# vlad17/runlmc

Measured on AMD Instinct MI355X. Metric: kronecker_toeplitz_mvms_per_sec, higher is better.
Workload: dtype f64

## Files before the change

runlmc_amd/csrc/rl_gridop.hip:

```cpp
#include "rl_host.h"

static thread_local std::string g_err;

int fail(int code, const std::string& msg) {
    g_err = msg;
    return code;
}

extern "C" const char* rl_last_error(void) { return g_err.c_str(); }
extern "C" const char* rl_backend(void) { return RL_BACKEND_NAME; }
extern "C" int rl_abi_version(void) { return RL_ABI_VERSION; }
extern "C" int rl_device_count(int* count) {
    if (!count) return fail(RL_EINVAL, "count is NULL");
    RL_HIP(hipGetDeviceCount(count));
    return RL_OK;
}

void trace_once(const char* what) {
    static const bool on = getenv("RUNLMC_TRACE") != nullptr;
    if (!on) return;
    static std::vector<std::string> seen;
    for (const std::string& s : seen)
        if (s == what) return;
    seen.push_back(what);
// ... 1 lines not shown
}

bool first_on_device(unsigned long long* seen) {
    int dev = 0;
    (void)hipGetDevice(&dev);
    const unsigned long long bit = 1ull << (dev & 63);
    if (*seen & bit) return false;
    *seen |= bit;
    return true;
}

RlKnobs read_knobs() {
    RlKnobs k;
    const char* dbg = getenv("RUNLMC_DEBUG");
    const bool debug = dbg != nullptr && dbg[0] != '\0' && dbg[0] != '0';
    auto ignored = [](const char* n) {
        static std::vector<std::string> told;
        if (std::find(told.begin(), told.end(), std::string(n)) == told.end()) {
            told.push_back(n);
            fprintf(stderr, "runlmc_hip: %s is a debug switch and is ignored without RUNLMC_DEBUG=1\n", n);
        }
    };
    auto user_flag = [](const char* n) { return getenv(n) != nullptr; };
    auto user_num = [](const char* n, long long dflt) {
        const char* e = getenv(n);
        return e ? atoll(e) : dflt;
    };
    auto flag = [&](const char* n) {
        if (getenv(n) == nullptr) return false;
        if (!debug) ignored(n);
        return debug;
    };
    auto num = [&](const char* n, long long dflt) {
        const char* e = getenv(n);
        if (e == nullptr) return dflt;
        if (!debug) ignored(n);
        return debug ? atoll(e) : dflt;
    };
    k.pow2_only = user_flag("RUNLMC_POW2_ONLY");
    k.chunk_mb = (int)num("RUNLMC_CHUNK_MB", 0);
    k.two_streams = (int)num("RUNLMC_TWO_STREAMS", -1);
    k.affine = (int)num("RUNLMC_AFFINE", -1);
    k.affine_kb = (int)num("RUNLMC_AFFINE_KB", 0);
    k.affine_max_kb = (int)num("RUNLMC_AFFINE_MAX_KB", 2048);
    k.no_v1p = flag("RUNLMC_NO_V1P");
    k.v1p_min = (int)num("RUNLMC_V1P_MIN", 0);
    k.no_lowrank = flag("RUNLMC_NO_LOWRANK");
    k.no_filter = flag("RUNLMC_NO_FILTER");
    k.no_lr_bound = flag("RUNLMC_NO_LR_BOUND");
    k.sf_carries1 = flag("RUNLMC_SF_CARRIES1");
    k.sf_scan2 = flag("RUNLMC_SF_SCAN2");
    k.poly_round = flag("RUNLMC_POLY_ROUND");
    k.no_poly_round = flag("RUNLMC_NO_POLY_ROUND");
    k.lr_min = num("RUNLMC_LR_MIN", -1);
    k.staged_wt = flag("RUNLMC_STAGED_WT");
    k.no_staged_wt = flag("RUNLMC_NO_STAGED_WT");
    k.no_w_poly = flag("RUNLMC_NO_W_POLY");
    k.no_rp = flag("RUNLMC_NO_RP");
    k.rp_stagger = (int)num("RUNLMC_RP_STAGGER", 7);
    k.no_lr_small = flag("RUNLMC_NO_LR_SMALL");
    k.no_precond_approx = flag("RUNLMC_NO_PRECOND_APPROX");
    k.no_precond_hi = flag("RUNLMC_NO_PRECOND_HI");
    k.precond_hi_passes = flag("RUNLMC_PRECOND_HI_PASSES");
    k.no_precond_hi_mixed = flag("RUNLMC_NO_PRECOND_HI_MIXED");
    k.precond_hi_min = num("RUNLMC_PRECOND_HI_MIN", 100000);
    k.precond_hi_rank = (int)num("RUNLMC_PRECOND_HI_RANK", 192);
    k.precond_hi_use = (int)num("RUNLMC_PRECOND_HI_USE", 0);
    k.rp_fly = (int)num("RUNLMC_RP_FLY", 1);
    k.no_rp_small = flag("RUNLMC_NO_RP_SMALL");
    k.no_rp_fuse = flag("RUNLMC_NO_RP_FUSE");
    k.rp_pfuse = !flag("RUNLMC_NO_RP_PFUSE");
    k.w_pfuse = !flag("RUNLMC_NO_W_PFUSE");
    k.rp_runlen = (int)num("RUNLMC_RP_RUNLEN", 0);
    k.w_poly_rmax = std::min(36, (int)num("RUNLMC_W_POLY_RMAX", 32));
    k.no_sort = flag("RUNLMC_NO_SORT");
    k.ws_cache_mb = user_num("RUNLMC_WS_CACHE_MB", -1);
    k.solver_maxblk = (int)num("RUNLMC_SOLVER_MAXBLK", 0);
    k.no_fuse_w = flag("RUNLMC_NO_FUSE_W");
    k.no_fuse_wt = flag("RUNLMC_NO_FUSE_WT");
    k.no_graph = flag("RUNLMC_NO_GRAPH");
#if defined(RL_EMU)
    k.minres_v1 = flag("RUNLMC_MINRES_V1");
#endif
    return k;
}

static int ilog2(int x) {
    int l = 0;
    while ((1 << l) < x) ++l;
    return l;
}

static FftPlan make_plan(int n) {
    FftPlan p;
    p.n = n;
    p.npass = 0;
    for (int i = 0; i < RL_MAX_PASSES; ++i) p.radix[i] = 1;
    int rem = n;
    for (int odd : {3, 5})
        while (rem % odd == 0 && p.npass < 2) {
            p.radix[p.npass++] = odd;
            rem /= odd;
        }
    const int fixed[7][4] = {{8, 8, 0, 0},     {16, 16, 0, 0},   {64, 8, 8, 0},
                             {128, 8, 16, 0},  {256, 16, 16, 0}, {512, 8, 8, 8},
                             {1024, 8, 8, 16}};
    for (const auto& f : fixed)
        if (f[0] == rem) {
            for (int i = 1; i < 4 && f[i]; ++i) p.radix[p.npass++] = f[i];
            return p;
        }
    while (rem > 1) {
        int r = 8;
        while (rem % r) r /= 2;
        p.radix[p.npass++] = r;
        rem /= r;
    }
    return p;
}

static bool make_plan_rows3(int n, FftPlan* p) {
    int ra, rb;
    switch (n) {
        case 128: ra = 8; rb = 8; break;
        case 256: ra = 16; rb = 8; break;
        case 512: ra = 16; rb = 16; break;
        default: return false;
    }
    p->n = n;
    p->npass = 3;
    for (int i = 0; i < RL_MAX_PASSES; ++i) p->radix[i] = 1;
    p->radix[0] = ra;
    p->radix[1] = rb;
    p->radix[2] = 2;
    return true;
}

static int fused_code(const FftPlan& p) {
    if (p.npass < 2 || p.npass > 4) return 0;
    const int ra = p.radix[0], rb = p.radix[p.npass - 1];
    const int code = ra * 100 + rb;
    switch (code) {
        case 808: case 816: case 1616: return p.n >= 64 ? code : 0;
        case 308: case 316: case 508: case 516: return code;
        default: return 0;
    }
}

static void choose_length(int m, bool pow2_only, int* L_out, int* N1_out, int* N2_out) {
    long best = 0;
    int best_odd = 1;
    for (int odd : {1, 3, 5, 9, 15, 25}) {
        if (odd != 1 && pow2_only) continue;
        long L = odd;
        while (L < 2L * m || L < 16) L *= 2;
        if (odd != 1 && L / odd < 64 * 8) continue;
        if (best == 0 || L < best) { best = L; best_odd = odd; }
    }
    const int L = (int)best;
    const int P = L / best_odd;
    const int l = ilog2(P);
    int N2 = 1 << ((l + 1) / 2);
    if (best_odd != 1) {
        int bestN2 = 0;
        double bestScore = 1e300;
        for (int n2 = 64; n2 <= 1024 && n2 <= P / 8; n2 *= 2) {
// ... 274 lines not shown
    if (((size_t)g->N1 * C + g->N1) * sizeof(cplx) > kLdsHard)
        return fail(RL_ELIMIT, "rl_gridop_create: grid too long for one LDS column tile");
    g->colsA = C;

    g->plan1 = make_plan(g->N1);
    g->plan2 = make_plan(g->N2);
    g->code1 = fused_code(g->plan1);
    g->code2 = fused_code(g->plan2);
    bool rows_ok = g->code2 == 808 || g->code2 == 816 || g->code2 == 1616;
    if (g->code1 != 0 &&
        (size_t)g->N2 * D * sizeof(cplx) <= kLdsHard && make_plan_rows3(g->N2, &g->plan2)) {
        g->rows3 = true;
        g->code2 = g->plan2.radix[0] * 100 + g->plan2.radix[1];
        rows_ok = true;
    }
    g->v2 = g->code1 != 0 && rows_ok;
    g->lr_try = m1 == 0 && m >= 2 * RL_LR_RMAX && m < (1 << 28) && !g->kn.no_lowrank;
    g->lr_round_try = g->lr_try && (m >= 2048 || g->kn.poly_round);
    g->sf_try = m1 == 0 && m >= 64 && !g->kn.no_filter;
    g->lr_min = lr_min_elements(g);
    g->h_freq1 = position_to_freq(g->plan1);
    g->h_freq2 = position_to_freq(g->plan2);

    int rc;
    if ((rc = upload(&g->tw1, unity_table(g->N1, 1, g->N1))) != RL_OK) return rc;
    if ((rc = upload(&g->tw2, unity_table(g->N2, 1, g->N2))) != RL_OK) return rc;
    const int shift = l / 2;
    if ((rc = upload(&g->twlo, unity_table(1L << shift, 1, L))) != RL_OK) return rc;
    if ((rc = upload(&g->twhi, unity_table(((long)L + (1L << shift) - 1) >> shift, 1L << shift,
                                           L))) != RL_OK) return rc;
    if ((rc = upload(&g->freq1, g->h_freq1)) != RL_OK) return rc;
    g->twl.lo = m1 == 0 ? g->twlo : nullptr;
    g->twl.hi = g->twhi;
    g->twl.shift = shift;
    g->twl.mask = (1 << shift) - 1;

    g->max_fac = max_tops * D;
    RL_HIP(hipMalloc((void**)&g->tops, (size_t)max_tops * m * sizeof(double)));
    RL_HIP(hipMalloc((void**)&g->spec, (size_t)max_tops * L * sizeof(double)));
    RL_HIP(hipMalloc((void**)&g->facA, (size_t)g->max_fac * D * sizeof(double)));
    RL_HIP(hipMalloc((void**)&g->facW, (size_t)g->max_fac * sizeof(double)));
    RL_HIP(hipMalloc((void**)&g->facQ, (size_t)g->max_fac * sizeof(int)));
    RL_HIP(hipMalloc((void**)&g->kappa, (size_t)max_tops * D * sizeof(double)));
    std::vector<double> ones(D, 1.0);
    if ((rc = upload(&g->ones, ones)) != RL_OK) return rc;

    size_t chunk_mb = (size_t)D * L * sizeof(cplx) >= ((size_t)8 << 20) ? 64 : 192;
    if (g->kn.chunk_mb > 0) chunk_mb = (size_t)g->kn.chunk_mb;
    g->chunk_pairs = std::max<size_t>(1, (chunk_mb << 20) / ((size_t)D * L * sizeof(cplx)));
    {
        const size_t pairT = (size_t)D * L * sizeof(cplx);
        const bool can = g->v2 && g->rows3 && m1 == 0;
        g->affine = can && (g->kn.affine >= 0 ? g->kn.affine != 0
                                              : (pairT >= ((size_t)512 << 10) &&
                                                 pairT <= ((size_t)g->kn.affine_max_kb << 10)));
        if (g->affine && g->kn.affine_kb > 0 && g->kn.chunk_mb <= 0)
            g->chunk_pairs = 8 * std::max<size_t>(1, ((size_t)g->kn.affine_kb << 10) / pairT);
    }
    if (m1 == 0 && L <= 2048 && !g->kn.no_v1p) {
        const size_t lds = ((size_t)L * (D | 1) + L) * sizeof(cplx);
        if (lds <= kLdsHard) {
            g->planL = make_plan(L);
            if ((rc = upload(&g->twL, unity_table(L, 1, L))) != RL_OK) return rc;
            RL_HIP(hipMalloc((void**)&g->spec1, (size_t)max_tops * L * sizeof(double)));
            g->lds1 = lds;
            g->thr1 = (size_t)D * L >= 4096 ? 512 : 256;
            g->v1p = true;
            if (g->kn.v1p_min > 0) g->v1p_min = g->kn.v1p_min;
        }
    }
    *out = guard.release();
    return RL_OK;
}

extern "C" int rl_gridop_destroy(rl_gridop* g) {
    if (!g) return RL_OK;
    (void)hipSetDevice(g->device);
    if (g->child) (void)rl_gridop_destroy(g->child);
    if (g->wide_B) (void)hipFree(g->wide_B);
    if (g->wide_Z) (void)hipFree(g->wide_Z);
    void* ptrs[] = {g->tw1, g->tw2, g->twlo, g->twhi, g->freq1, g->tops, g->spec,
                    g->facA, g->facW, g->facQ, g->kappa, g->ones, g->T,
                    g->T2[0], g->T2[1], g->T2[2], g->twL, g->spec1, g->mixtab, g->lr_beta, g->lr_nu, g->lr_phiJ, g->lr_stat, g->lr_M,
                    g->lr_B, g->lr_eye, g->lr_part, g->lr_zhat, g->lr_scr, g->lr_pw, g->lr_sel, g->lr_Cc, g->lr_Bc, g->lr_Mf, g->lr_spart, g->lr_Cx,
                    g->sf_tops, g->sf_blob, g->sf_blob_top, g->sf_pwp, g->sf_pw, g->sf_kappa, g->sf_facA, g->sf_facAW, g->sf_facJ,
                    g->sf_E, g->sf_Cin, g->sf_next};
    for (void* p : ptrs)
        if (p) (void)hipFree(p);
    if (g->ev_fork) (void)hipEventDestroy(g->ev_fork);
    for (int i = 0; i < 3; ++i) {
        if (g->ev_join[i]) (void)hipEventDestroy(g->ev_join[i]);
        if (g->aux[i]) (void)hipStreamDestroy(g->aux[i]);
    }
    delete g;
    return RL_OK;
}

extern "C" int rl_gridop_info(const rl_gridop* g, int* L, int* N1, int* N2, int* colsA,
                              int* rowsB) {
    if (!g) return fail(RL_EINVAL, "gridop is NULL");
    if (L) *L = g->L;
    if (N1) *N1 = g->N1;
    if (N2) *N2 = g->N2;
    if (colsA) *colsA = g->colsA;
    if (rowsB) *rowsB = g->rowsB;
    return RL_OK;
}

extern "C" int rl_gridop_form(const rl_gridop* gc, int* rank, long long* min_elements) {
    if (!gc) return fail(RL_EINVAL, "gridop is NULL");
    if (gc->wide) {
        return rl_gridop_form(gc->child, rank, min_elements);
    }
    rl_gridop* g = const_cast<rl_gridop*>(gc);
    if (g->Q >= 1) RL_TRY(lr_ensure(g));
    if (rank) *rank = g->lr_ok ? g->lr_r : 0;
    if (min_elements) *min_elements = (long long)g->lr_min;
    return RL_OK;
}

extern "C" int rl_gridop_top_forms(const rl_gridop* gc, int* forms, int* structured) {
    if (!gc) return fail(RL_EINVAL, "gridop is NULL");
    if (gc->wide) {
        RL_TRY(rl_gridop_top_forms(gc->child, forms, nullptr));
        if (structured) {
            *structured = 1;
            for (int q = 0; q < gc->child->Q; ++q)
                if (gc->child->top_form[q] == 0) *structured = 0;
        }
        return RL_OK;
    }
    rl_gridop* g = const_cast<rl_gridop*>(gc);
    if (g->Q < 1) return fail(RL_EINVAL, "grid operator has no parameters yet");
    RL_TRY(lr_ensure(g));
    if (forms)
        for (int q = 0; q < g->Q; ++q)
            forms[q] = q < (int)g->top_form.size() ? g->top_form[q] : 0;
    if (structured) *structured = (g->lr_ok || g->st_ok) ? 1 : 0;
    return RL_OK;
}

extern "C" int rl_gridop_form_stats(const rl_gridop* gc, int q, double* out4) {
    if (!gc || !out4) return fail(RL_EINVAL, "rl_gridop_form_stats: NULL argument");
    if (gc->wide) return rl_gridop_form_stats(gc->child, q, out4);
    rl_gridop* g = const_cast<rl_gridop*>(gc);
    if (g->Q < 1) return fail(RL_EINVAL, "grid operator has no parameters yet");
    if (q < 0 || q >= g->Q) return fail(RL_EINVAL, "rl_gridop_form_stats: no such top row");
    RL_TRY(lr_ensure(g));
    for (int k = 0; k < 4; ++k)
        out4[k] = (size_t)(4 * q + k) < g->lr_vstat.size() ? g->lr_vstat[4 * q + k] : 0.0;
    return RL_OK;
}

extern "C" int rl_gridop_set_form_gate(rl_gridop* g, long long min_elements) {
    if (!g) return fail(RL_EINVAL, "gridop is NULL");
    if (g->wide) return rl_gridop_set_form_gate(g->child, min_elements);
    g->lr_min = min_elements < 0 ? lr_min_elements(g) : (size_t)min_elements;
    return RL_OK;
}

static int build_spectra(rl_gridop* g, int ntop, hipStream_t stream) {
    const int npairs = (ntop + 1) / 2;
    const size_t need = ((size_t)npairs + g->D - 1) / g->D;
    RL_TRY(ensure_workspace(g, std::max<size_t>(need, 1)));
    dim3 gridA(g->N2 / g->colsA, 1, npairs);
    Gather no_gather;
    no_gather.indptr = nullptr;
// ... 495 lines not shown
    std::vector<double> phiJ((size_t)(R + 16) * m, 0.0), beta(R), nu(R);
    std::vector<long double> prev(m, 0.0L), cur(m), nxt(m);
    const long double p0 = 1.0L / sqrtl((long double)m);
    for (int n = 0; n < m; ++n) cur[n] = p0;
    long double bj = 0.0L, nuj = p0;
    for (int j = 0; j < R + RL_LR_EXTRA; ++j) {
        for (int n = 0; n < m; ++n) phiJ[(size_t)j * m + n] = (double)cur[n];
        if (j < R) {
            beta[j] = (double)(bj * bj);
            nu[j] = (double)nuj;
        }
        long double nrm = 0.0L;
        for (int n = 0; n < m; ++n) {
            const long double sn = m > 1 ? -1.0L + 2.0L * n / (m - 1) : 0.0L;
            nxt[n] = sn * cur[n] - bj * prev[n];
            nrm += nxt[n] * nxt[n];
        }
        bj = sqrtl(nrm);
        if (!(bj > 0.0L)) return fail(RL_EINVAL, "polynomial basis degenerate");
        nuj /= bj;
        for (int n = 0; n < m; ++n) {
            prev[n] = cur[n];
            cur[n] = nxt[n] / bj;
        }
    }
    RL_TRY(upload(&g->lr_phiJ, phiJ));
    RL_TRY(upload(&g->lr_beta, beta));
    RL_TRY(upload(&g->lr_nu, nu));
    g->lr_hnu = nu;
    return RL_OK;
}

static int lr_steps(const rl_gridop* g, int nrows, int R) {
    const int slots = (g->m + 1) / 2;
    if (slots <= 64 * RL_LR_T) return std::max(4, ((slots + 63) / 64 + 3) / 4 * 4);
    const int rowblocks = (nrows + RL_LR_ROWS(R) - 1) / RL_LR_ROWS(R);
    const double resident = 2.0 * RL_LR_CUS;
    int best = RL_LR_T;
    double best_cost = 1e300;
    for (int steps = RL_LR_T; steps <= 8 * RL_LR_T; steps *= 2) {
        const int chunks = ((g->m + 1) / 2 + 64 * steps - 1) / (64 * steps);
        const double rounds = std::ceil((double)chunks * rowblocks / resident);
        const double cost = rounds * (steps + 8);
        if (cost < best_cost * 0.97) {
            best_cost = cost;
            best = steps;
        }
        if (chunks == 1) break;
    }
    return best;
}
static int lr_nchunks_max(const rl_gridop* g) {
    return ((g->m + 1) / 2 + 64 * RL_LR_T - 1) / (64 * RL_LR_T);
}
static size_t lr_part_need(const rl_gridop* g, int nvec) {
    return (size_t)lr_nchunks_max(g) * nvec * g->D * RL_LR_RMAX;
}
int lr_reserve(rl_gridop* g, int nvec) {
    const size_t rows = (size_t)nvec * g->D;
    const size_t need_part = lr_part_need(g, nvec), need_z = rows * RL_LR_RMAX;
    if (g->lr_part_cap < need_part) {
        if (g->lr_part) RL_HIP(hipFree(g->lr_part));
        g->lr_part = nullptr;
        g->lr_part_cap = 0;
        RL_HIP(hipMalloc((void**)&g->lr_part, need_part * sizeof(double)));
        g->lr_part_cap = need_part;
    }
    if (g->lr_zhat_cap < need_z) {
        if (g->lr_zhat) RL_HIP(hipFree(g->lr_zhat));
        g->lr_zhat = nullptr;
        g->lr_zhat_cap = 0;
        RL_HIP(hipMalloc((void**)&g->lr_zhat, need_z * sizeof(double)));
        g->lr_zhat_cap = need_z;
    }
    return RL_OK;
}

static size_t lr_min_elements(const rl_gridop* g) {
    return g->kn.lr_min >= 0 ? (size_t)g->kn.lr_min : (size_t)1 << 20;
}

template <int R>
static int lr_project(rl_gridop* g, const double* X, int nrows, hipStream_t st,
                      double* part = nullptr) {
    const int steps = lr_steps(g, nrows, R);
    const int chunks = ((g->m + 1) / 2 + 64 * steps - 1) / (64 * steps);
    RL_LAUNCH((k_lr_project<R>), dim3(chunks, (nrows + RL_LR_ROWS(R) - 1) / RL_LR_ROWS(R)),
              dim3(64 * RL_LR_WAVES), (size_t)RL_LR_WAVES * R * 65 * sizeof(double), st, X, nrows,
              g->m, (const double*)g->lr_beta, steps, part != nullptr ? part : g->lr_part);
    return chunks;
}
template <int R>
static void lr_mix(rl_gridop* g, const double* part, int chunks, int nvec, int Q, const double* Cq,
                   const double* Bq, double* zhat, hipStream_t st) {
    int split3 = 0;
    const size_t mix_lds = lr_mix_lds(g->D, R, Q, &split3);
    RL_LAUNCH(k_lr_mix, dim3(nvec), dim3(RL_LR_MIXT), mix_lds, st, part, chunks, nvec, g->D, R, Q,
              Cq, Bq, (const double*)g->lr_nu, zhat, (const int*)nullptr, split3);
}
template <int R>
static void lr_expand(rl_gridop* g, const double* zhat, int nrows, double* Y, int accumulate,
                      hipStream_t st) {
    const int per_cu = 8;
    const int nbx = ((g->m + 1) / 2 + 255) / 256;
    int rpb = 16;
    if ((size_t)nbx * ((nrows + 15) / 16) < (size_t)2 * per_cu * RL_LR_CUS) {
        const int nby = std::max(1, std::min(nrows, per_cu * RL_LR_CUS / nbx));
        rpb = (nrows + nby - 1) / nby;
    }
    if (accumulate)
        RL_LAUNCH((k_lr_expand<R, true>), dim3(nbx, (nrows + rpb - 1) / rpb), dim3(256), 0,
                  st, zhat, nrows, g->m, (const double*)g->lr_beta, rpb, Y);
    else
        RL_LAUNCH((k_lr_expand<R, false>), dim3(nbx, (nrows + rpb - 1) / rpb), dim3(256), 0,
                  st, zhat, nrows, g->m, (const double*)g->lr_beta, rpb, Y);
}
template <int R>
static void lr_launch(rl_gridop* g, const double* X, double* Y, int nvec, int Q, const double* Cq,
                      const double* Bq, hipStream_t st, int accumulate = 0) {
    const int nrows = nvec * g->D;
    const bool deferred = g->defer_expand && !accumulate && R <= g->kn.w_poly_rmax;
    const int chunks = lr_project<R>(g, X, nrows, st);
    lr_mix<R>(g, g->lr_part, chunks, nvec, Q, Cq, Bq, g->lr_zhat, st);
    if (deferred) {
        g->expand_deferred = true;
        return;
    }
    lr_expand<R>(g, g->lr_zhat, nrows, Y, accumulate, st);
}

static int lr_apply(rl_gridop* g, const double* X, double* Y, int nvec, int q0, int Q,
                    const double* Bq, hipStream_t st) {
    const double* Cq = g->lr_C + (size_t)q0 * g->lr_r * g->lr_r;
    switch (g->lr_r) {
        case 24: lr_launch<24>(g, X, Y, nvec, Q, Cq, Bq, st); break;
        case 32: lr_launch<32>(g, X, Y, nvec, Q, Cq, Bq, st); break;
        case 36: lr_launch<36>(g, X, Y, nvec, Q, Cq, Bq, st); break;
        case 40: lr_launch<40>(g, X, Y, nvec, Q, Cq, Bq, st); break;
        case 48: lr_launch<48>(g, X, Y, nvec, Q, Cq, Bq, st); break;
        default: return fail(RL_EINVAL, "low-rank path: bad basis size");
    }
    RL_HIP(hipGetLastError());
    return RL_OK;
}

static int lr_apply_compact(rl_gridop* g, const double* X, double* Y, int nvec, hipStream_t st) {
    switch (g->lr_r) {
        case 24: lr_launch<24>(g, X, Y, nvec, g->lr_np, g->lr_Cc, g->lr_Bc, st, 1); break;
        case 32: lr_launch<32>(g, X, Y, nvec, g->lr_np, g->lr_Cc, g->lr_Bc, st, 1); break;
        case 36: lr_launch<36>(g, X, Y, nvec, g->lr_np, g->lr_Cc, g->lr_Bc, st, 1); break;
        case 40: lr_launch<40>(g, X, Y, nvec, g->lr_np, g->lr_Cc, g->lr_Bc, st, 1); break;
        case 48: lr_launch<48>(g, X, Y, nvec, g->lr_np, g->lr_Cc, g->lr_Bc, st, 1); break;
        default: return fail(RL_EINVAL, "low-rank path: bad basis size");
    }
    RL_HIP(hipGetLastError());
    return RL_OK;
}

static int mvm_with_mix(rl_gridop* g, const MixParams& mp, const double* X, double* Y, int nvec,
                        hipStream_t stream);

struct SfFit {
    int deg = 0;
    long double ah = 0.0L;
    long double c[3] = {0.0L, 0.0L, 0.0L};
};

static bool sf_check(const double* t, int m, const SfFit& f, long double tot) {
// ... 252 lines not shown
            red[512 + tid] += red[512 + tid + s];
        }
        __syncthreads();
    }
    if (tid == 0) {
        out[blockIdx.x * 3 + 0] = red[0];
        out[blockIdx.x * 3 + 1] = red[256];
        out[blockIdx.x * 3 + 2] = red[512];
    }
}
__global__ void __launch_bounds__(256)
k_lr_rowmax(const double* __restrict__ V, int m, double* __restrict__ out) {
    RL_SMEM(smem);
    double* red = reinterpret_cast<double*>(smem);
    const double* v = V + (size_t)blockIdx.x * m;
    double mx = 0.0;
    for (int i = threadIdx.x; i < m; i += 256) {
        const double a = fabs(v[i]);
        mx = (a > mx || !(a <= 1e300)) ? a : mx;
    }
    const int tid = threadIdx.x;
    red[tid] = mx;
    __syncthreads();
    for (int s = 128; s > 0; s >>= 1) {
        if (tid < s) {
            const double o = red[tid + s];
            if (o > red[tid] || !(o <= 1e300)) red[tid] = o;
        }
        __syncthreads();
    }
    if (tid == 0) out[blockIdx.x] = red[0];
}
#define RL_LR_NPOW 8
#define RL_LR_TOL_OP 2e-13
#if defined(RL_EMU)
#define RL_LR_PWB 8
#else
#define RL_LR_PWB 512
#endif
__global__ void __launch_bounds__(256)
k_lr_pw_diff(const double* a, const double* b, int m, double* out, double* __restrict__ part) {
    RL_SMEM(smem);
    double* red = reinterpret_cast<double*>(smem);
    const size_t off = (size_t)blockIdx.y * m;
    double s = 0.0;
    for (int i = blockIdx.x * 256 + threadIdx.x; i < m; i += gridDim.x * 256) {
        const double d = b ? a[off + i] - b[off + i] : a[off + i];
        out[off + i] = d;
        s = fma(d, d, s);
    }
    const int tid = threadIdx.x;
    red[tid] = s;
    __syncthreads();
    for (int w = 128; w > 0; w >>= 1) {
        if (tid < w) red[tid] += red[tid + w];
        __syncthreads();
    }
    if (tid == 0) part[(size_t)blockIdx.y * gridDim.x + blockIdx.x] = red[0];
}
__global__ void __launch_bounds__(256)
k_lr_pw_scale(const double* __restrict__ d, int m, const double* __restrict__ part,
              double* __restrict__ v, double* __restrict__ stat, const int* __restrict__ top_of_row,
              int stride, int off) {
    RL_SMEM(smem);
    double* red = reinterpret_cast<double*>(smem);
    const int row = blockIdx.y, tid = threadIdx.x;
    double sp = 0.0;
    for (int b = tid; b < (int)gridDim.x; b += 256) sp += part[(size_t)row * gridDim.x + b];
    red[tid] = sp;
    __syncthreads();
    for (int w = 128; w > 0; w >>= 1) {
        if (tid < w) red[tid] += red[tid + w];
        __syncthreads();
    }
    const double nrm = sqrt(red[0]);
    const double inv = (nrm > 0.0 && nrm <= 1e300) ? 1.0 / nrm : 1.0;
    const size_t o = (size_t)row * m;
    for (int i = blockIdx.x * 256 + threadIdx.x; i < m; i += gridDim.x * 256) v[o + i] = d[o + i] * inv;
    if (blockIdx.x == 0 && threadIdx.x == 0 && top_of_row[row] >= 0)
        stat[(size_t)top_of_row[row] * stride + off] = nrm;
}
#define RL_LR_STATW (RL_LR_NB * 3 + RL_LR_RMAX + 16 + 2 * RL_LR_NPOW)

static int lr_verify(rl_gridop* g, const std::vector<char>& want, std::vector<char>* pass) {
    const int D = g->D, m = g->m, Q = g->Q;
    const size_t vec = (size_t)D * m;
    pass->assign(Q, 0);
    if (!g->lr_phiJ) {
        RL_TRY(lr_make_basis(g));
        double* cs = nullptr;
        RL_HIP(hipMalloc((void**)&cs, (size_t)g->max_tops * (RL_LR_STATW + RL_LR_RMAX * RL_LR_RMAX) * sizeof(double)));
        RL_HIP(hipMemset(cs, 0, (size_t)g->max_tops * (RL_LR_STATW + RL_LR_RMAX * RL_LR_RMAX) * sizeof(double)));
        g->lr_stat = cs;
        g->lr_C = cs + (size_t)g->max_tops * RL_LR_STATW;
        RL_HIP(hipMalloc((void**)&g->lr_Cc, (size_t)g->max_tops * RL_LR_RMAX * RL_LR_RMAX * sizeof(double)));
        RL_HIP(hipMalloc((void**)&g->lr_B, (size_t)g->max_tops * D * D * sizeof(double)));
        RL_HIP(hipMalloc((void**)&g->lr_Bc, (size_t)g->max_tops * D * D * sizeof(double)));
        std::vector<double> eye((size_t)D * D, 0.0);
        for (int a = 0; a < D; ++a) eye[(size_t)a * D + a] = 1.0;
        RL_TRY(upload(&g->lr_eye, eye));
        const size_t nvr = (RL_LR_RMAX + RL_LR_EXTRA + D - 1) / D;
        RL_HIP(hipMalloc((void**)&g->lr_scr, (3 + nvr) * vec * sizeof(double)));
        RL_HIP(hipMalloc((void**)&g->lr_pw, (4 * vec + 2 * (size_t)RL_LR_PWB * D) * sizeof(double)));
        RL_HIP(hipMalloc((void**)&g->lr_sel, (size_t)g->max_tops *
                         ((size_t)g->max_tops * D + (size_t)g->max_tops * D * D + D) * sizeof(double)));
        std::vector<double> xr(vec);
        unsigned long long st = 0x9E3779B97F4A7C15ull;
        for (size_t i = 0; i < vec; ++i) {
            st = st * 6364136223846793005ull + 1442695040888963407ull;
            xr[i] = ((double)(st >> 11) / 9007199254740992.0) * 2.0 - 1.0;
        }
        for (int a = 0; a < D; ++a) {
            long double ss = 0.0L;
            for (int i = 0; i < m; ++i) ss += (long double)xr[(size_t)a * m + i] * xr[(size_t)a * m + i];
            const double inv = ss > 0.0L ? (double)(1.0L / sqrtl(ss)) : 1.0;
            for (int i = 0; i < m; ++i) xr[(size_t)a * m + i] *= inv;
        }
        RL_HIP(hipMemcpy(g->lr_scr, xr.data(), vec * sizeof(double), hipMemcpyHostToDevice));
    }
    double* xr = g->lr_scr;
    double* y1 = xr + vec;
    double* y2 = y1 + vec;
    double* tphi = y2 + vec;
    hipStream_t st = nullptr;
    std::vector<double> back;
    std::vector<char> best;
    std::vector<int> cand;
    for (int q = 0; q < Q; ++q)
        if (want[q]) cand.push_back(q);
    const size_t sel_stride = (size_t)Q * D + (size_t)Q * D * D + D;
    {
        const size_t ngroups = (cand.size() + D - 1) / D;
        std::vector<double> sel(std::max<size_t>(1, ngroups) * sel_stride, 0.0);
        for (size_t grp = 0; grp < ngroups; ++grp) {
            double* ks = sel.data() + grp * sel_stride;
            double* bs = ks + (size_t)Q * D;
            int* rows = reinterpret_cast<int*>(bs + (size_t)Q * D * D);
            for (int a = 0; a < D; ++a) rows[a] = -1;
            for (int a = 0; a < D && grp * D + a < cand.size(); ++a) {
                const int q = cand[grp * D + a];
                ks[(size_t)q * D + a] = 1.0;
                bs[((size_t)q * D + a) * D + a] = 1.0;
                rows[a] = q;
            }
        }
        RL_HIP(hipMemcpy(g->lr_sel, sel.data(), sel.size() * sizeof(double), hipMemcpyHostToDevice));
    }
    for (int r : {24, 32, 36, 40, 48}) {
        if (r < g->lr_rank_hint && r < 48) continue;
        g->lr_r = r;
        const int nvr = (r + RL_LR_EXTRA + D - 1) / D, nrows = nvr * D;
        RL_TRY(lr_reserve(g, std::max(nvr, 1)));
        RL_HIP(hipMemsetAsync(g->lr_C, 0, (size_t)g->max_tops * RL_LR_RMAX * RL_LR_RMAX * sizeof(double), st));
        for (int q = 0; q < Q; ++q) {
            if (!want[q]) continue;
            MixParams mp{1, 0, g->spec + (size_t)q * g->L, nullptr, nullptr, nullptr, g->ones,
                         nullptr, nullptr};
            double* stat = g->lr_stat + (size_t)q * RL_LR_STATW;
            g->lr_bypass = true;
            int rc = mvm_with_mix(g, mp, g->lr_phiJ, tphi, nvr, st);
            g->lr_bypass = false;
            if (rc != RL_OK) return rc;
            RL_LAUNCH(k_lr_rowmax, dim3(nrows), dim3(256), 256 * sizeof(double), st,
                      (const double*)tphi, m, stat + RL_LR_NB * 3);
            int nparts = 0;
            switch (r) {
                case 24: nparts = lr_project<24>(g, tphi, nrows, st); break;
                case 32: nparts = lr_project<32>(g, tphi, nrows, st); break;
                case 36: nparts = lr_project<36>(g, tphi, nrows, st); break;
                case 40: nparts = lr_project<40>(g, tphi, nrows, st); break;
                default: nparts = lr_project<48>(g, tphi, nrows, st); break;
            }
            RL_LAUNCH(k_lr_finish_C, dim3(r), dim3(256), 512 * sizeof(double), st,
                      (const double*)g->lr_part, nparts, nrows, r, (const double*)g->lr_nu,
                      g->lr_C + (size_t)q * r * r);
            g->lr_bypass = true;
            rc = mvm_with_mix(g, mp, xr, y1, 1, st);
            g->lr_bypass = false;
            if (rc != RL_OK) return rc;
            RL_TRY(lr_apply(g, xr, y2, 1, q, 1, g->lr_eye, st));
            RL_LAUNCH(k_lr_compare, dim3(RL_LR_NB), dim3(256), 3 * 256 * sizeof(double), st,
                      (const double*)y1, (const double*)y2, vec, stat);
        }
        for (size_t grp = 0; grp * D < cand.size(); ++grp) {
            double* vw = g->lr_pw;
            double* Tvw = vw + 2 * vec;
            double* parts = Tvw + 2 * vec;
            const double* ksel = g->lr_sel + grp * sel_stride;
            const double* bsel = ksel + (size_t)Q * D;
            const int* rows = reinterpret_cast<const int*>(bsel + (size_t)Q * D * D);
            MixParams mps{Q, 0, g->spec, nullptr, nullptr, nullptr, ksel, nullptr, nullptr};
            RL_HIP(hipMemcpyAsync(vw, xr, vec * sizeof(double), hipMemcpyDeviceToDevice, st));
            RL_HIP(hipMemcpyAsync(vw + vec, xr, vec * sizeof(double), hipMemcpyDeviceToDevice, st));
            const int recE = RL_LR_NB * 3 + RL_LR_RMAX + 16;
            for (int k = 0; k < RL_LR_NPOW; ++k) {
                g->lr_bypass = true;
                int rc = mvm_with_mix(g, mps, vw, Tvw, 2, st);
                g->lr_bypass = false;
                if (rc != RL_OK) return rc;
                RL_TRY(lr_apply(g, vw, y2, 1, 0, Q, bsel, st));
                const dim3 pg(RL_LR_PWB, D);
                RL_LAUNCH(k_lr_pw_diff, pg, dim3(256), 256 * sizeof(double), st, (const double*)Tvw,
                          (const double*)y2, m, Tvw, parts);
                RL_LAUNCH(k_lr_pw_scale, pg, dim3(256), 256 * sizeof(double), st, (const double*)Tvw, m,
                          (const double*)parts, vw, g->lr_stat, rows, RL_LR_STATW, recE + k);
                RL_LAUNCH(k_lr_pw_diff, pg, dim3(256), 256 * sizeof(double), st,
                          (const double*)(Tvw + vec), (const double*)nullptr, m, Tvw + vec,
                          parts + (size_t)RL_LR_PWB * D);
                RL_LAUNCH(k_lr_pw_scale, pg, dim3(256), 256 * sizeof(double), st,
                          (const double*)(Tvw + vec), m, (const double*)(parts + (size_t)RL_LR_PWB * D),
                          vw + vec, g->lr_stat, rows, RL_LR_STATW, recE + RL_LR_NPOW + k);
            }
        }
        RL_HIP(hipGetLastError());
        back.resize((size_t)g->max_tops * RL_LR_STATW + (size_t)Q * r * r);
        RL_HIP(hipMemcpy(back.data(), g->lr_stat, back.size() * sizeof(double), hipMemcpyDeviceToHost));
        std::vector<char> ok(Q, 0);
        bool all = true;
        for (int q = 0; q < Q; ++q) {
            if (!want[q]) continue;
            const double* stat = back.data() + (size_t)q * RL_LR_STATW;
            double dmax = 0.0, ymax = 0.0, bad = 0.0;
            for (int b = 0; b < RL_LR_NB; ++b) {
                dmax = std::max(dmax, stat[b * 3]);
                ymax = std::max(ymax, stat[b * 3 + 1]);
                bad += stat[b * 3 + 2];
            }
            const double* rm = stat + RL_LR_NB * 3;
            double inside = 0.0, outside = 0.0;
            bool finite = bad == 0.0 && std::isfinite(ymax);
            for (int j = 0; j < r + RL_LR_EXTRA; ++j) {
                if (!std::isfinite(rm[j])) finite = false;
                (j < r ? inside : outside) = std::max(j < r ? inside : outside, rm[j]);
            }
            const bool trial = dmax <= RL_LR_TOL * ymax || (ymax == 0.0 && dmax == 0.0);
            const bool tail = outside <= RL_LR_TOL * inside || (inside == 0.0 && outside == 0.0);
            const double* rec = rm + RL_LR_RMAX + 16;
            double sigE = 0.0, sigT = 0.0;
            for (int k = 0; k < RL_LR_NPOW; ++k) {
                if (!std::isfinite(rec[k]) || !std::isfinite(rec[RL_LR_NPOW + k])) finite = false;
                sigE = std::max(sigE, rec[k]);
                sigT = std::max(sigT, rec[RL_LR_NPOW + k]);
            }
            const bool bound = g->kn.no_lr_bound || sigE <= RL_LR_TOL_OP * sigT || (sigE == 0.0 && sigT == 0.0);
            if ((int)g->lr_vstat.size() < 4 * g->max_tops) g->lr_vstat.assign((size_t)4 * g->max_tops, 0.0);
            g->lr_vstat[4 * q + 0] = ymax > 0.0 ? dmax / ymax : dmax;
            g->lr_vstat[4 * q + 1] = inside > 0.0 ? outside / inside : outside;
            g->lr_vstat[4 * q + 2] = sigE;
            g->lr_vstat[4 * q + 3] = sigT;
            ok[q] = finite && trial && tail && bound;
            all = all && ok[q];
        }
        best = ok;
        if (all) break;
    }
    *pass = best;
    const int r = g->lr_r;
    g->lr_hC.assign(back.begin() + (size_t)g->max_tops * RL_LR_STATW,
                    back.begin() + (size_t)g->max_tops * RL_LR_STATW + (size_t)Q * r * r);
    return RL_OK;
}

static int forms_setup(rl_gridop* g, const std::vector<double>& A, const std::vector<double>& W,
                       const std::vector<int>& Qi, const std::vector<double>& kap) {
    const int D = g->D, m = g->m, Q = g->Q;
    g->lr_ok = false;
    g->st_ok = false;
    g->top_form.assign(Q, 0);
    g->sf_slot.assign(Q, -1);
    g->sf_top_ns.assign(Q, 2);
    g->sf_n = 0;
    g->sf_nfac = 0;
    g->lr_np = 0;
    if (!g->lr_try && !g->sf_try) return RL_OK;
    std::vector<double> B((size_t)Q * D * D, 0.0);
    for (size_t f = 0; f < W.size(); ++f)
        for (int a = 0; a < D; ++a)
            for (int b = 0; b < D; ++b)
                B[((size_t)Qi[f] * D + a) * D + b] += W[f] * A[f * D + a] * A[f * D + b];
    for (int q = 0; q < Q; ++q)
        for (int a = 0; a < D; ++a) B[((size_t)q * D + a) * D + a] += kap[(size_t)q * D + a];
    g->lr_hB = B;
    std::vector<SfFit> fits(Q);
// ... 582 lines not shown
```

runlmc_amd/csrc/rl_host.h:

```cpp
#pragma once
#include "../../include/runlmc_hip.h"

#include <algorithm>
#include <cmath>
#include <cstdio>
#include <cstdlib>
#include <cstring>
#include <functional>
#include <string>
#include <thread>
#include <vector>

#include "rl_kernels.h"
#include "rl_kernels2.h"
#include "rl_kernels3.h"
#include "rl_lowrank.h"
#include "rl_rowpoly.h"
#include "rl_filter.h"

#define RL_MAX_D 16

int fail(int code, const std::string& msg);
#define RL_HIP(expr)                                                                   \
    do {                                                                               \
        hipError_t e_ = (expr);                                                        \
        if (e_ != hipSuccess)                                                          \
            return fail(RL_EHIP, std::string(#expr) + ": " + hipGetErrorString(e_));   \
    } while (0)

#define RL_TRY(expr)              \
    do {                          \
        int rc_ = (expr);         \
        if (rc_ != RL_OK) return rc_; \
    } while (0)


void trace_once(const char* what);
bool first_on_device(unsigned long long* seen);

struct RlKnobs {
    bool pow2_only = false;
    int chunk_mb = 0;
    int two_streams = -1;
    int affine = -1;
    int affine_kb = 0;
    int affine_max_kb = 2048;
    bool no_v1p = false;
    int v1p_min = 0;
    bool no_lowrank = false;
    bool no_filter = false;
    bool sf_scan2 = false;
    bool sf_carries1 = false;
    bool no_lr_bound = false;
    bool poly_round = false;
    bool no_poly_round = false;
    long long lr_min = -1;
    bool staged_wt = false;
    bool no_staged_wt = false;
    bool no_w_poly = false;
    bool no_rp = false;
    int rp_stagger = 7;
    int rp_runlen = 0;
    bool no_rp_small = false;
    bool rp_pfuse = true;
    bool w_pfuse = true;
    bool no_rp_fuse = false;
    bool no_lr_small = false;
    bool no_precond_approx = false;
    long long precond_hi_min = 100000;
    int precond_hi_use = 0;
    int precond_hi_rank = 192;
    bool no_precond_hi_mixed = false;
    bool precond_hi_passes = false;
    bool no_precond_hi = false;
    int rp_fly = 1;
    int w_poly_rmax = 32;
    bool no_sort = false;
    long long ws_cache_mb = -1;
    int solver_maxblk = 0;
    bool no_fuse_w = false;
    bool no_fuse_wt = false;
    bool no_graph = false;
    bool minres_v1 = false;
};
RlKnobs read_knobs();

template <class T>
static int upload(T** dev, const std::vector<T>& host) {
    RL_HIP(hipMalloc((void**)dev, std::max<size_t>(host.size(), 1) * sizeof(T)));
    if (!host.empty())
        RL_HIP(hipMemcpy(*dev, host.data(), host.size() * sizeof(T), hipMemcpyHostToDevice));
    return RL_OK;
}

static const size_t kLdsSoft = 76 * 1024;
static const size_t kLdsHard = 156 * 1024;

struct rl_gridop {
    RlKnobs kn;
    int device = 0;
    int D = 0, m = 0, L = 0, N1 = 0, N2 = 0;
    Geom geo{0, 0, 0};
    int colsA = 0;
    int rowsB = 0;
    int rowsS = 0;
    int code1 = 0, code2 = 0;
    bool v2 = false;
    bool rows3 = false;
    bool lr_try = false;
    bool lr_ok = false;
    bool lr_round_try = false;
    bool wide = false;
    rl_gridop* child = nullptr;
    double* wide_B = nullptr;
    double* wide_Z = nullptr;
    size_t wide_Z_cap = 0;
    bool defer_expand = false;
    bool expand_deferred = false;
    int lr_rejects = 0;
    int lr_skip = 0;
    double* lr_stat = nullptr;
    bool lr_dirty = false;
    std::vector<double> lr_A, lr_W, lr_kap;
    std::vector<int> lr_Qi;
    bool lr_bypass = false;
    int lr_r = 0;
    int lr_rank_hint = 0;
    size_t lr_min = 0;
    double* lr_beta = nullptr;
    double* lr_nu = nullptr;
    double* lr_phiJ = nullptr;
    double* lr_C = nullptr;
    double* lr_M = nullptr;
    std::vector<double> lr_hC;
    double* lr_spart = nullptr;
    size_t lr_spart_cap = 0;
    double* lr_Cx = nullptr;
    double* lr_Mf = nullptr;
    size_t lr_Mf_cap = 0;
    bool lr_Mf_ok = false;
    std::vector<double> lr_hB;
    std::vector<double> lr_hnu;
    unsigned long long param_ver = 0;
    double* lr_B = nullptr;
    double* lr_eye = nullptr;
    double* lr_part = nullptr;
    size_t lr_part_cap = 0;
    double* lr_zhat = nullptr;
    size_t lr_zhat_cap = 0;
    double* lr_scr = nullptr;
    double* lr_pw = nullptr;
    double* lr_sel = nullptr;
    std::vector<double> lr_vstat;
    double* lr_Cc = nullptr;
    double* lr_Bc = nullptr;
    int lr_np = 0;
    std::vector<double> h_tops;
    std::vector<int> top_form;
    bool st_ok = false;
    bool sf_try = false;
    int sf_n = 0;
    int sf_nfac = 0;
    int sf_ns = 2;
    std::vector<int> sf_slot;
    std::vector<int> sf_top_ns;
    SfTop* sf_tops = nullptr;
    double* sf_pwp = nullptr;
    double* sf_blob = nullptr;
    double* sf_blob_top = nullptr;
    double* sf_pw = nullptr;
    double* sf_kappa = nullptr;
    double* sf_facA = nullptr;
    double* sf_facAW = nullptr;
    int* sf_facJ = nullptr;
    double* sf_E = nullptr;
    size_t sf_E_cap = 0;
    double* sf_Cin = nullptr;
    int* sf_next = nullptr;
    size_t sf_Cin_cap = 0;
    double* mixtab = nullptr;
    size_t mixtab_rows = 0;
    bool mixtab_ok = false;
    int max_tops = 0;
    FftPlan plan1, plan2;
    cplx *tw1 = nullptr, *tw2 = nullptr, *twlo = nullptr, *twhi = nullptr;
    int* freq1 = nullptr;
    TwiddleL twl;
    std::vector<int> h_freq1, h_freq2;
    int Q = 0, nfac = 0;
    double* tops = nullptr;
    double* spec = nullptr;
    double* facA = nullptr;
    double* facW = nullptr;
    int* facQ = nullptr;
    double* kappa = nullptr;
    double* ones = nullptr;
    int max_fac = 0;
    cplx* T = nullptr;
    size_t T_pairs = 0;
    cplx* T2[3] = {nullptr, nullptr, nullptr};
    size_t T2_pairs = 0;
    int nside = 0;
    cplx* Tcur = nullptr;
    hipStream_t aux[3] = {nullptr, nullptr, nullptr};
    hipEvent_t ev_fork = nullptr, ev_join[3] = {nullptr, nullptr, nullptr};
    size_t chunk_pairs = 1;
    bool affine = false;
    bool v1p = false;
    FftPlan planL;
    cplx* twL = nullptr;
    double* spec1 = nullptr;
    size_t lds1 = 0;
    int thr1 = 256;
    int v1p_min = 64;
};

struct SkiTerm {
    rl_gridop* g = nullptr;
    int ngrid = 0;
    int *W_indptr = nullptr, *W_indices = nullptr;
    double* W_data = nullptr;
    int *WT_indptr = nullptr, *WT_indices = nullptr;
    double* WT_data = nullptr;
    int nnzWT = 0;
    int* W4_base = nullptr;
    double* W4_w = nullptr;
    int* WT_lo = nullptr;
    int wt_xmax = 0, wt_emax = 0;
    int w_xmax = 0;
    std::vector<int> h_base;
};

struct SolverWork {
    double* vec[10] = {nullptr, nullptr, nullptr, nullptr, nullptr,
                       nullptr, nullptr, nullptr, nullptr, nullptr};
// ... 159 lines not shown
```

Baseline: 260,200.

## Batch low-rank verification across candidate kernels instead of per-q serial launches

The low-rank verification step now runs every candidate kernel's basis MVMs into one shared buffer. It then does the rowmax, projection, C finish and comparison as single batched launches indexed by candidate. The power-iteration diff and scale kernels also gain a z dimension so both vectors are processed in one launch. This cuts kernel launch count and serial work during setup, at the cost of a larger scratch allocation, and the old serial path stays available behind an env flag. Verification is setup work, so the effect on steady-state MVM throughput is unclear.

```diff
diff --git a/runlmc_amd/csrc/rl_gridop.hip b/runlmc_amd/csrc/rl_gridop.hip
--- a/runlmc_amd/csrc/rl_gridop.hip
+++ b/runlmc_amd/csrc/rl_gridop.hip
@@ -107,6 +107,7 @@
 #if defined(RL_EMU)
     k.minres_v1 = flag("RUNLMC_MINRES_V1");
 #endif
+    k.lr_verify_serial = flag("RUNLMC_LR_VERIFY_SERIAL");
     return k;
 }
 
@@ -547,7 +548,7 @@
     void* ptrs[] = {g->tw1, g->tw2, g->twlo, g->twhi, g->freq1, g->tops, g->spec,
                     g->facA, g->facW, g->facQ, g->kappa, g->ones, g->T,
                     g->T2[0], g->T2[1], g->T2[2], g->twL, g->spec1, g->mixtab, g->lr_beta, g->lr_nu, g->lr_phiJ, g->lr_stat, g->lr_M,
-                    g->lr_B, g->lr_eye, g->lr_part, g->lr_zhat, g->lr_scr, g->lr_pw, g->lr_sel, g->lr_Cc, g->lr_Bc, g->lr_Mf, g->lr_spart, g->lr_Cx,
+                    g->lr_B, g->lr_eye, g->lr_part, g->lr_zhat, g->lr_scr, g->lr_pw, g->lr_sel, g->lr_bout, g->lr_cand, g->lr_Cc, g->lr_Bc, g->lr_Mf, g->lr_spart, g->lr_Cx,
                     g->sf_tops, g->sf_blob, g->sf_blob_top, g->sf_pwp, g->sf_pw, g->sf_kappa, g->sf_facA, g->sf_facAW, g->sf_facJ,
                     g->sf_E, g->sf_Cin, g->sf_next};
     for (void* p : ptrs)
@@ -1209,8 +1210,8 @@
 
 template <int R>
 static int lr_project(rl_gridop* g, const double* X, int nrows, hipStream_t st,
-                      double* part = nullptr) {
-    const int steps = lr_steps(g, nrows, R);
+                      double* part = nullptr, int steps = 0) {
+    if (steps <= 0) steps = lr_steps(g, nrows, R);
     const int chunks = ((g->m + 1) / 2 + 64 * steps - 1) / (64 * steps);
     RL_LAUNCH((k_lr_project<R>), dim3(chunks, (nrows + RL_LR_ROWS(R) - 1) / RL_LR_ROWS(R)),
               dim3(64 * RL_LR_WAVES), (size_t)RL_LR_WAVES * R * 65 * sizeof(double), st, X, nrows,
@@ -1629,6 +1630,135 @@
 }
 #define RL_LR_STATW (RL_LR_NB * 3 + RL_LR_RMAX + 16 + 2 * RL_LR_NPOW)
 
+__global__ void __launch_bounds__(256)
+k_lr_rowmax_sel(const double* __restrict__ V, int m, int per, const int* __restrict__ cand,
+                double* __restrict__ stat) {
+    RL_SMEM(smem);
+    double* red = reinterpret_cast<double*>(smem);
+    const int c = blockIdx.x / per, j = blockIdx.x % per;
+    const double* x = V + (size_t)blockIdx.x * m;
+    double mx = 0.0;
+    for (int i = threadIdx.x; i < m; i += 256) {
+        const double e = fabs(x[i]);
+        mx = (e > mx || !(e <= 1e300)) ? e : mx;
+    }
+    const int tid = threadIdx.x;
+    red[tid] = mx;
+    __syncthreads();
+    for (int s = 128; s > 0; s >>= 1) {
+        if (tid < s) {
+            const double o = red[tid + s];
+            if (o > red[tid] || !(o <= 1e300)) red[tid] = o;
+        }
+        __syncthreads();
+    }
+    if (tid == 0 && j < RL_LR_RMAX + 16) stat[(size_t)cand[c] * RL_LR_STATW + RL_LR_NB * 3 + j] = red[0];
+}
+__global__ void __launch_bounds__(256)
+k_lr_finish_C_sel(const double* __restrict__ part, int nparts, int nrows, int r,
+                  const double* __restrict__ nu, int per, const int* __restrict__ cand,
+                  double* __restrict__ C) {
+    RL_SMEM(smem);
+    double* red = reinterpret_cast<double*>(smem);
+    const int i = blockIdx.x, c = blockIdx.y, j = threadIdx.x & 63, cls = threadIdx.x >> 6;
+    const size_t r0 = (size_t)c * per;
+    double a = 0.0, b = 0.0;
+    if (j < r)
+        for (int p = cls; p < nparts; p += 4) {
+            a += part[((size_t)p * nrows + r0 + j) * r + i];
+            b += part[((size_t)p * nrows + r0 + i) * r + j];
+        }
+    red[cls * 64 + j] = a;
+    red[256 + cls * 64 + j] = b;
+    __syncthreads();
+    if (cls == 0 && j < r) {
+        a = (red[j] + red[64 + j]) + (red[128 + j] + red[192 + j]);
+        b = (red[256 + j] + red[320 + j]) + (red[384 + j] + red[448 + j]);
+        C[(size_t)cand[c] * r * r + i * r + j] = 0.5 * (nu[i] * a + nu[j] * b);
+    }
+}
+__global__ void __launch_bounds__(256)
+k_lr_compare_sel(const double* __restrict__ Y1, const double* __restrict__ Y2, size_t n,
+                 const int* __restrict__ cand, double* __restrict__ stat) {
+    RL_SMEM(smem);
+    double* red = reinterpret_cast<double*>(smem);
+    const double* y1 = Y1 + (size_t)blockIdx.y * n;
+    const double* y2 = Y2 + (size_t)blockIdx.y * n;
+    double dmax = 0.0, ymax = 0.0, bad = 0.0;
+    for (size_t i = (size_t)blockIdx.x * 256 + threadIdx.x; i < n; i += (size_t)gridDim.x * 256) {
+        const double a = y1[i], b = y2[i], d = fabs(a - b);
+        if (!(d <= 1e300)) bad += 1.0;
+        else dmax = d > dmax ? d : dmax;
+        ymax = fabs(a) > ymax ? fabs(a) : ymax;
+    }
+    const int tid = threadIdx.x;
+    red[tid] = dmax;
+    red[256 + tid] = ymax;
+    red[512 + tid] = bad;
+    __syncthreads();
+    for (int s = 128; s > 0; s >>= 1) {
+        if (tid < s) {
+            red[tid] = red[tid] > red[tid + s] ? red[tid] : red[tid + s];
+            red[256 + tid] = red[256 + tid] > red[256 + tid + s] ? red[256 + tid] : red[256 + tid + s];
+            red[512 + tid] += red[512 + tid + s];
+        }
+        __syncthreads();
+    }
+    if (tid == 0) {
+        double* out = stat + (size_t)cand[blockIdx.y] * RL_LR_STATW + blockIdx.x * 3;
+        out[0] = red[0];
+        out[1] = red[256];
+        out[2] = red[512];
+    }
+}
+__global__ void __launch_bounds__(256)
+k_lr_pw_diff2(double* Tvw, const double* __restrict__ y2, int m, size_t vec,
+              double* __restrict__ parts) {
+    RL_SMEM(smem);
+    double* red = reinterpret_cast<double*>(smem);
+    const int z = blockIdx.z;
+    double* out = Tvw + z * vec + (size_t)blockIdx.y * m;
+    const double* b = z == 0 ? y2 + (size_t)blockIdx.y * m : nullptr;
+    double s = 0.0;
+    for (int i = blockIdx.x * 256 + threadIdx.x; i < m; i += gridDim.x * 256) {
+        const double d = b ? out[i] - b[i] : out[i];
+        out[i] = d;
+        s = fma(d, d, s);
+    }
+    const int tid = threadIdx.x;
+    red[tid] = s;
+    __syncthreads();
+    for (int w = 128; w > 0; w >>= 1) {
+        if (tid < w) red[tid] += red[tid + w];
+        __syncthreads();
+    }
+    if (tid == 0)
+        parts[(size_t)z * gridDim.x * gridDim.y + (size_t)blockIdx.y * gridDim.x + blockIdx.x] = red[0];
+}
+__global__ void __launch_bounds__(256)
+k_lr_pw_scale2(const double* __restrict__ Tvw, int m, size_t vec, const double* __restrict__ parts,
+               double* __restrict__ vw, double* __restrict__ stat, const int* __restrict__ top_of_row,
+               int stride, int offE, int offT) {
+    RL_SMEM(smem);
+    double* red = reinterpret_cast<double*>(smem);
+    const int row = blockIdx.y, z = blockIdx.z, tid = threadIdx.x;
+    const double* part = parts + (size_t)z * gridDim.x * gridDim.y;
+    double sp = 0.0;
+    for (int b = tid; b < (int)gridDim.x; b += 256) sp += part[(size_t)row * gridDim.x + b];
+    red[tid] = sp;
+    __syncthreads();
+    for (int w = 128; w > 0; w >>= 1) {
+        if (tid < w) red[tid] += red[tid + w];
+        __syncthreads();
+    }
+    const double nrm = sqrt(red[0]);
+    const double inv = (nrm > 0.0 && nrm <= 1e300) ? 1.0 / nrm : 1.0;
+    const size_t o = z * vec + (size_t)row * m;
+    for (int i = blockIdx.x * 256 + threadIdx.x; i < m; i += gridDim.x * 256) vw[o + i] = Tvw[o + i] * inv;
+    if (blockIdx.x == 0 && threadIdx.x == 0 && top_of_row[row] >= 0)
+        stat[(size_t)top_of_row[row] * stride + (z ? offT : offE)] = nrm;
+}
+
 static int lr_verify(rl_gridop* g, const std::vector<char>& want, std::vector<char>* pass) {
     const int D = g->D, m = g->m, Q = g->Q;
     const size_t vec = (size_t)D * m;
@@ -1693,13 +1823,61 @@
         }
         RL_HIP(hipMemcpy(g->lr_sel, sel.data(), sel.size() * sizeof(double), hipMemcpyHostToDevice));
     }
+    const bool serial = g->kn.lr_verify_serial;
+    const int ncand = (int)cand.size();
+    if (!serial && ncand > 0) {
+        if (!g->lr_cand) RL_HIP(hipMalloc((void**)&g->lr_cand, (size_t)g->max_tops * sizeof(int)));
+        RL_HIP(hipMemcpy(g->lr_cand, cand.data(), cand.size() * sizeof(int), hipMemcpyHostToDevice));
+    }
     for (int r : {24, 32, 36, 40, 48}) {
         if (r < g->lr_rank_hint && r < 48) continue;
         g->lr_r = r;
         const int nvr = (r + RL_LR_EXTRA + D - 1) / D, nrows = nvr * D;
         RL_TRY(lr_reserve(g, std::max(nvr, 1)));
         RL_HIP(hipMemsetAsync(g->lr_C, 0, (size_t)g->max_tops * RL_LR_RMAX * RL_LR_RMAX * sizeof(double), st));
-        for (int q = 0; q < Q; ++q) {
+        if (!serial && ncand > 0) {
+            const int nvr = (r + RL_LR_EXTRA + D - 1) / D, per = nvr * D, nrows = ncand * per;
+            const size_t need = (size_t)ncand * (nvr + 2);
+            if (g->lr_bcap < need) {
+                if (g->lr_bout) RL_HIP(hipFree(g->lr_bout));
+                g->lr_bout = nullptr;
+                g->lr_bcap = 0;
+                RL_HIP(hipMalloc((void**)&g->lr_bout, need * vec * sizeof(double)));
+                g->lr_bcap = need;
+            }
+            RL_TRY(lr_reserve(g, ncand * nvr));
+            double* tb = g->lr_bout;
+            double* t1 = tb + (size_t)ncand * nvr * vec;
+            double* t2 = t1 + (size_t)ncand * vec;
+            for (int c = 0; c < ncand; ++c) {
+                const int q = cand[c];
+                MixParams mp{1, 0, g->spec + (size_t)q * g->L, nullptr, nullptr, nullptr, g->ones,
+                             nullptr, nullptr};
+                g->lr_bypass = true;
+                int rc = mvm_with_mix(g, mp, g->lr_phiJ, tb + (size_t)c * nvr * vec, nvr, st);
+                if (rc == RL_OK) rc = mvm_with_mix(g, mp, xr, t1 + (size_t)c * vec, 1, st);
+                g->lr_bypass = false;
+                if (rc != RL_OK) return rc;
+            }
+            RL_LAUNCH(k_lr_rowmax_sel, dim3(nrows), dim3(256), 256 * sizeof(double), st,
+                      (const double*)tb, m, per, (const int*)g->lr_cand, g->lr_stat);
+            int nparts = 0;
+            switch (r) {
+                case 24: nparts = lr_project<24>(g, tb, nrows, st, nullptr, lr_steps(g, per, 24)); break;
+                case 32: nparts = lr_project<32>(g, tb, nrows, st, nullptr, lr_steps(g, per, 32)); break;
+                case 36: nparts = lr_project<36>(g, tb, nrows, st, nullptr, lr_steps(g, per, 36)); break;
+                case 40: nparts = lr_project<40>(g, tb, nrows, st, nullptr, lr_steps(g, per, 40)); break;
+                default: nparts = lr_project<48>(g, tb, nrows, st, nullptr, lr_steps(g, per, 48)); break;
+            }
+            RL_LAUNCH(k_lr_finish_C_sel, dim3(r, ncand), dim3(256), 512 * sizeof(double), st,
+                      (const double*)g->lr_part, nparts, nrows, r, (const double*)g->lr_nu, per,
+                      (const int*)g->lr_cand, g->lr_C);
+            for (int c = 0; c < ncand; ++c)
+                RL_TRY(lr_apply(g, xr, t2 + (size_t)c * vec, 1, cand[c], 1, g->lr_eye, st));
+            RL_LAUNCH(k_lr_compare_sel, dim3(RL_LR_NB, ncand), dim3(256), 3 * 256 * sizeof(double), st,
+                      (const double*)t1, (const double*)t2, vec, (const int*)g->lr_cand, g->lr_stat);
+        }
+        for (int q = 0; serial && q < Q; ++q) {
             if (!want[q]) continue;
             MixParams mp{1, 0, g->spec + (size_t)q * g->L, nullptr, nullptr, nullptr, g->ones,
                          nullptr, nullptr};
@@ -1746,6 +1924,14 @@
                 g->lr_bypass = false;
                 if (rc != RL_OK) return rc;
                 RL_TRY(lr_apply(g, vw, y2, 1, 0, Q, bsel, st));
+                if (!serial) {
+                    RL_LAUNCH(k_lr_pw_diff2, dim3(RL_LR_PWB, D, 2), dim3(256), 256 * sizeof(double), st,
+                              Tvw, (const double*)y2, m, vec, parts);
+                    RL_LAUNCH(k_lr_pw_scale2, dim3(RL_LR_PWB, D, 2), dim3(256), 256 * sizeof(double), st,
+                              (const double*)Tvw, m, vec, (const double*)parts, vw, g->lr_stat, rows,
+                              RL_LR_STATW, recE + k, recE + RL_LR_NPOW + k);
+                    continue;
+                }
                 const dim3 pg(RL_LR_PWB, D);
                 RL_LAUNCH(k_lr_pw_diff, pg, dim3(256), 256 * sizeof(double), st, (const double*)Tvw,
                           (const double*)y2, m, Tvw, parts);
diff --git a/runlmc_amd/csrc/rl_host.h b/runlmc_amd/csrc/rl_host.h
--- a/runlmc_amd/csrc/rl_host.h
+++ b/runlmc_amd/csrc/rl_host.h
@@ -82,6 +82,7 @@
     bool no_fuse_wt = false;
     bool no_graph = false;
     bool minres_v1 = false;
+    bool lr_verify_serial = false;
 };
 RlKnobs read_knobs();
 
@@ -151,6 +152,9 @@
     double* lr_scr = nullptr;
     double* lr_pw = nullptr;
     double* lr_sel = nullptr;
+    double* lr_bout = nullptr;
+    size_t lr_bcap = 0;
+    int* lr_cand = nullptr;
     std::vector<double> lr_vstat;
     double* lr_Cc = nullptr;
     double* lr_Bc = nullptr;
```

Result: no change. 259,600 (median of 6 runs) (-0.2%).
